# grantjr1842/delayed-streams-modeling

Hardware: AMD Instinct MI355X
Metric: real-time stream throughput, stt-1b-en_fr @ bs=64 per GPU (Mimi encode + LM decode per 80 ms frame) (higher is better)
Workload: dtype bf16 weights + bf16 KV, f32 activations as three exact bf16 pieces, f32 accumulate (v_mfma_f32_16x16x32_bf16); 1 GPU; stt-1b-en_fr batch=64 streaming, ring KV cache full (750 frames), Mimi encode + LM decode HIP path; streams_per_gpu=64, parallelism=replicas x1 (independent stream batches, no per-step collective), streams=encoder stream || 2 LM group stream(s)

## Files before the change

delayed-streams-modeling_amd/csrc/dsm_engine_api.inc:

```

namespace {

template <typename KVT, int HD, int T>
int launch_attn_t(dsm_engine* e, hipStream_t st, float* out, const float* q, const void* k, const void* v,
                  const uint32_t* start_pos, const uint8_t* active, int B, int H, int ctx, int d, const AttnFused& fq) {
  size_t lds = sizeof(float) * ((size_t)T * ctx + 4 * T * HD + 16);
  if ((long)B * H >= 2048 && (size_t)2 * ctx * HD * sizeof(KVT) >= (size_t)256 * 1024) lds += e->attn_lds_pad;
  if (lds > 64 * 1024) {
    static size_t allowed = 0;
    if (lds > allowed) {
      HIPCHK(hipFuncSetAttribute(reinterpret_cast<const void*>(&attn_kernel<KVT, HD, T, 8>), hipFuncAttributeMaxDynamicSharedMemorySize, (int)lds));
      HIPCHK(hipFuncSetAttribute(reinterpret_cast<const void*>(&attn_kernel<KVT, HD, T, 4>), hipFuncAttributeMaxDynamicSharedMemorySize, (int)lds));
      allowed = lds;
    }
  }
  const int tag = e->tag_attn[e->sid(st)];
  if (T == 1 && HD == 64 && ctx <= 32 && e->attn_small) {
    const int ph = e->prof_begin(tag, st);
    hipLaunchKernelGGL((attn_small_kernel<KVT, 64>), dim3((B * H + 3) / 4), dim3(256), 0, st, out, q, reinterpret_cast<const KVT*>(k),
                       reinterpret_cast<const KVT*>(v), start_pos, active, B * H, H, ctx, d, fq);
    e->prof_end(ph, st);
    HIPCHK(hipGetLastError());
    return 0;
  }
  const int ph = e->prof_begin(tag, st);
  const bool unr8 = sizeof(KVT) == 2 && T == 1 && (e->attn_unr == 8 || (e->attn_unr == 0 && HD == 128));
  if (unr8)
    hipLaunchKernelGGL((attn_kernel<KVT, HD, T, 8>), dim3(B * H), dim3(256), lds, st, out, q, reinterpret_cast<const KVT*>(k),
                       reinterpret_cast<const KVT*>(v), start_pos, active, H, ctx, d, e->dev_ts_slot(tag, e->sid(st), 0), fq);
  else
    hipLaunchKernelGGL((attn_kernel<KVT, HD, T, 4>), dim3(B * H), dim3(256), lds, st, out, q, reinterpret_cast<const KVT*>(k),
                       reinterpret_cast<const KVT*>(v), start_pos, active, H, ctx, d, e->dev_ts_slot(tag, e->sid(st), 0), fq);
  e->prof_end(ph, st);
  HIPCHK(hipGetLastError());
  return 0;
}

template <typename KVT>
int launch_attn(dsm_engine* e, hipStream_t st, float* out, const float* q, const void* k, const void* v,
                const uint32_t* start_pos, const uint8_t* active, int B, int H, int hd, int T, int ctx, int d,
                const AttnFused& fq) {
#define DSM_ATTN(HDv, Tv) \
  if (hd == HDv && T == Tv) return launch_attn_t<KVT, HDv, Tv>(e, st, out, q, k, v, start_pos, active, B, H, ctx, d, fq);
  DSM_ATTN(32, 1) DSM_ATTN(64, 1) DSM_ATTN(128, 1) DSM_ATTN(32, 2) DSM_ATTN(64, 2) DSM_ATTN(128, 2)
#undef DSM_ATTN
  e->set_error("unsupported attention shape head_dim=%d T=%d (head_dim must be 32, 64 or 128; T 1 or 2)", hd, T);
  return DSM_ERR_INVALID;
}

int make_stream(dsm_engine* e, hipStream_t* st, int prio, int kind) {
  const int n = e->enc_cus;
  if (n <= 0 || n >= 32 || (kind == 2 && !e->lm_cus_excl)) {
    HIPCHK(hipStreamCreateWithPriority(st, hipStreamNonBlocking, prio));
    return 0;
  }
  uint32_t mask[8];
  for (int w = 0; w < 8; ++w) {
    uint32_t m = 0;
    for (int b = 0; b < 32; ++b) {
      const int cu = (32 * w + b) / 8;
      if ((kind == 1) == (cu < n)) m |= 1u << b;
    }
    mask[w] = m;
  }
  HIPCHK(hipExtStreamCreateWithCUMask(st, 8, mask));
  return 0;
}

int run_norm(dsm_engine* e, hipStream_t st, float* y, const float* x, const float* w, const float* b, int rows, int d,
             int rms) {
  hipLaunchKernelGGL(row_norm_kernel, dim3(rows), dim3(256), 0, st, y, x, w, b, rows, d,
                     rms ? 1e-8f : 1e-5f, rms);
  HIPCHK(hipGetLastError());
  return 0;
}

template <typename WT, typename KVT>
int transformer_forward(dsm_engine* e, hipStream_t st, const TransformerW& w, TransformerState& s, float* x, float* xn,
                        float* q, float* att, float* ff, int B, int T, const uint8_t* d_mask, float* final_out,
                        RowMap final_map, const float* post_norm_w = nullptr, float* post_norm_out = nullptr, int phase = 0,
                        const CaState* ca = nullptr, bool head_done = false) {
  const dsm_transformer_config& c = w.cfg;
  const int d = c.d_model, H = c.num_heads, hd = d / H, M = B * T;
  const float eps = c.norm == 1 ? 1e-8f : 1e-5f;
  if (phase != 2 && !head_done) {
    hipLaunchKernelGGL(kv_builder_kernel, dim3(B), dim3(64), 0, st, s.pos, s.idx, d_mask, s.start_pos, s.widx,
                       c.positional_embedding == 1 ? s.rope_cs : (float*)nullptr, w.inv_freq, B, T, c.context, hd,
                       w.rope_pos_before ? 1 : 0);
    HIPCHK(hipGetLastError());
// ... 1525 lines not shown
```

delayed-streams-modeling_amd/csrc/dsm_kernels.h:

```cpp
#pragma once
#include <hip/hip_runtime.h>
#include <stdint.h>
#include "dsm_numerics.h"
#include "dsm_sampling.h"

typedef float f32x4 __attribute__((ext_vector_type(4)));
typedef short dsm_bf16x8 __attribute__((ext_vector_type(8)));

__device__ __forceinline__ float wave_sum64(float v) {
#pragma unroll
  for (int off = 32; off >= 1; off >>= 1) v = v + __shfl_xor(v, off, 64);
  return v;
}

enum { EPI_STORE = 0, EPI_QKV = 1, EPI_GATE = 2, EPI_RVQ = 3 };

struct RowMap {
  long bstride;
  int rpb;
  int ld;
  int toff;
  __host__ __device__ long off(int m) const { return (long)(m / rpb) * bstride + (long)((m % rpb) + toff) * ld; }
};

struct GemmArgs {
  const float* X;
  RowMap xmap;
  const void* W;
  int Kpad, K, N, M;
  int nt_stride;
  int wpacked;
  int w_ntiles;
  int wg_cols;
  const float* bias;
  const float* scale;
  const float* res;
  RowMap rmap;
  float* Y;
  RowMap ymap;
  float* Y2;
  RowMap y2map;
  int act;
  int vec;
  int d, hd, H, T, ctx;
  void* kcache;
  void* vcache;
  const uint32_t* widx;
  const float* rope_cs;
  const uint8_t* active;
  float* pval;
  uint32_t* pidx;
  float* ws;
  int ws_ntiles;
  int defer_reduce;
  int chunk_loop;
  const float* norm_w;
  const float* norm_b;
  float* norm_out;
  float norm_eps;
  int norm_rms;
  int wk_hint;
  const float* pre_norm_w;
  const float* pre_norm_b;
  float pre_norm_eps;
  int pre_norm_rms;
  unsigned long long* ts;
};

template <typename WT>
__device__ __forceinline__ const WT* dsm_wbase(const GemmArgs& a, const WT* W, int n0, int r, int q) {
  if (sizeof(WT) == 2 && a.wpacked) return W + ((long)(n0 >> 4) * (a.Kpad >> 5)) * 512 + (q * 16 + r) * 8;
  return W + (long)(n0 + r) * a.Kpad + 8 * q;
}
template <typename WT>
__device__ __forceinline__ int dsm_wstep(const GemmArgs& a) { return (sizeof(WT) == 2 && a.wpacked) ? 16 : 1; }

__device__ __forceinline__ void launch_stamp_begin(unsigned long long* ts) {
  if (!ts || threadIdx.x != 0) return;
  const unsigned lin = blockIdx.x + gridDim.x * (blockIdx.y + gridDim.y * blockIdx.z);
  if (lin < 128) atomicMin(&ts[0], wall_clock64());
}
__device__ __forceinline__ void launch_stamp_end(unsigned long long* ts) {
  if (!ts || threadIdx.x != 0) return;
  const unsigned total = gridDim.x * gridDim.y * gridDim.z;
  const unsigned lin = blockIdx.x + gridDim.x * (blockIdx.y + gridDim.y * blockIdx.z);
  if (lin + 512 >= total) atomicMax(&ts[1], wall_clock64());
}

template <typename WT>
__device__ __forceinline__ void load_w8(const WT* p, float (&o)[8]);
template <>
__device__ __forceinline__ void load_w8<uint16_t>(const uint16_t* p, float (&o)[8]) {
  uint4 v = *reinterpret_cast<const uint4*>(p);
  o[0] = __uint_as_float(v.x << 16); o[1] = __uint_as_float(v.x & 0xFFFF0000u);
  o[2] = __uint_as_float(v.y << 16); o[3] = __uint_as_float(v.y & 0xFFFF0000u);
  o[4] = __uint_as_float(v.z << 16); o[5] = __uint_as_float(v.z & 0xFFFF0000u);
  o[6] = __uint_as_float(v.w << 16); o[7] = __uint_as_float(v.w & 0xFFFF0000u);
}
template <>
__device__ __forceinline__ void load_w8<float>(const float* p, float (&o)[8]) {
  float4 a = *reinterpret_cast<const float4*>(p);
  float4 b = *reinterpret_cast<const float4*>(p + 4);
  o[0] = a.x; o[1] = a.y; o[2] = a.z; o[3] = a.w; o[4] = b.x; o[5] = b.y; o[6] = b.z; o[7] = b.w;
}

template <typename KVT>
struct Raw8;
typedef unsigned int dsm_u32x4 __attribute__((ext_vector_type(4)));
typedef float dsm_f32x4v __attribute__((ext_vector_type(4)));
template <>
struct Raw8<uint16_t> {
  uint4 v;
  __device__ __forceinline__ void load(const uint16_t* p) { v = *reinterpret_cast<const uint4*>(p); }
  __device__ __forceinline__ void load_nt(const uint16_t* p) {
    const dsm_u32x4 t = __builtin_nontemporal_load(reinterpret_cast<const dsm_u32x4*>(p));
    v = make_uint4(t[0], t[1], t[2], t[3]);
  }
  __device__ __forceinline__ void unpack(float (&o)[8]) const {
    o[0] = __uint_as_float(v.x << 16); o[1] = __uint_as_float(v.x & 0xFFFF0000u);
    o[2] = __uint_as_float(v.y << 16); o[3] = __uint_as_float(v.y & 0xFFFF0000u);
    o[4] = __uint_as_float(v.z << 16); o[5] = __uint_as_float(v.z & 0xFFFF0000u);
    o[6] = __uint_as_float(v.w << 16); o[7] = __uint_as_float(v.w & 0xFFFF0000u);
  }
};
template <>
struct Raw8<float> {
  float4 a, b;
  __device__ __forceinline__ void load(const float* p) {
    a = *reinterpret_cast<const float4*>(p);
    b = *reinterpret_cast<const float4*>(p + 4);
  }
  __device__ __forceinline__ void load_nt(const float* p) {
    const dsm_f32x4v t0 = __builtin_nontemporal_load(reinterpret_cast<const dsm_f32x4v*>(p));
    const dsm_f32x4v t1 = __builtin_nontemporal_load(reinterpret_cast<const dsm_f32x4v*>(p + 4));
    a = make_float4(t0[0], t0[1], t0[2], t0[3]);
    b = make_float4(t1[0], t1[1], t1[2], t1[3]);
  }
  __device__ __forceinline__ void unpack(float (&o)[8]) const {
    o[0] = a.x; o[1] = a.y; o[2] = a.z; o[3] = a.w; o[4] = b.x; o[5] = b.y; o[6] = b.z; o[7] = b.w;
  }
};

__device__ __forceinline__ void store_kv(uint16_t* p, float v) { *p = dsm_f32_to_bf16(v); }
__device__ __forceinline__ void store_kv(float* p, float v) { *p = v; }

__device__ __forceinline__ void store_kv4(uint16_t* p, const float (&o)[4]) {
  uint2 v;
  v.x = (uint32_t)dsm_f32_to_bf16(o[0]) | ((uint32_t)dsm_f32_to_bf16(o[1]) << 16);
  v.y = (uint32_t)dsm_f32_to_bf16(o[2]) | ((uint32_t)dsm_f32_to_bf16(o[3]) << 16);
  *reinterpret_cast<uint2*>(p) = v;
}
__device__ __forceinline__ void store_kv4(float* p, const float (&o)[4]) {
  *reinterpret_cast<float4*>(p) = make_float4(o[0], o[1], o[2], o[3]);
}

template <typename KVT, int EPI>
__device__ __forceinline__ void epi_store_qkv(const GemmArgs& a, f32x4 v, int m, int n) {
  if (m >= a.M || n >= a.N) return;
  const bool full = a.vec && (n + 3 < a.N);
  if (EPI == EPI_STORE) {
    float o[4];
#pragma unroll
    for (int i = 0; i < 4; ++i) {
      float t = v[i];
      if (n + i < a.N) {
        if (a.bias) t = t + a.bias[n + i];
        if (a.act == 1) t = dsm_gelu_erf(t);
        if (a.scale) t = t * a.scale[n + i];
      }
      o[i] = t;
    }
    if (a.res) {
      const float* rp = a.res + a.rmap.off(m) + n;
      if (full) {
        float4 rv = *reinterpret_cast<const float4*>(rp);
        o[0] = rv.x + o[0]; o[1] = rv.y + o[1]; o[2] = rv.z + o[2]; o[3] = rv.w + o[3];
      } else {
#pragma unroll
        for (int i = 0; i < 4; ++i)
          if (n + i < a.N) o[i] = rp[i] + o[i];
      }
    }
    if (a.Y) {
      float* y = a.Y + a.ymap.off(m) + n;
      if (full) {
        *reinterpret_cast<float4*>(y) = make_float4(o[0], o[1], o[2], o[3]);
      } else {
#pragma unroll
        for (int i = 0; i < 4; ++i)
          if (n + i < a.N) y[i] = o[i];
      }
    }
    if (a.Y2) {
      float* y2 = a.Y2 + a.y2map.off(m) + n;
      if (full) {
        *reinterpret_cast<float4*>(y2) = make_float4(dsm_elu(o[0]), dsm_elu(o[1]), dsm_elu(o[2]), dsm_elu(o[3]));
      } else {
#pragma unroll
        for (int i = 0; i < 4; ++i)
          if (n + i < a.N) y2[i] = dsm_elu(o[i]);
      }
    }
  } else {
    const int part = n / a.d, c = n - part * a.d, h = c / a.hd, i0 = c - h * a.hd;
    const int b = m / a.T;
    float o[4] = {v[0], v[1], v[2], v[3]};
    if (part < 2 && a.rope_cs) {
      const float4 cs = *reinterpret_cast<const float4*>(a.rope_cs + ((long)m * (a.hd / 2) + (i0 >> 1)) * 2);
      const float co[2] = {cs.x, cs.z}, si[2] = {cs.y, cs.w};
#pragma unroll
      for (int p = 0; p < 2; ++p) {
        float x0 = v[2 * p], x1 = v[2 * p + 1];
        float t0 = x0 * co[p], t1 = x1 * si[p], t2 = x0 * si[p], t3 = x1 * co[p];
        o[2 * p] = t0 - t1;
        o[2 * p + 1] = t2 + t3;
      }
    }
    if (part == 0) {
      *reinterpret_cast<float4*>(a.Y + (long)m * a.d + c) = make_float4(o[0], o[1], o[2], o[3]);
    } else if (a.active[b]) {
      KVT* cache = reinterpret_cast<KVT*>(part == 1 ? a.kcache : a.vcache);
      store_kv4(cache + (((long)b * a.H + h) * a.ctx + a.widx[m]) * a.hd + i0, o);
// ... 501 lines not shown
    for (int nt = 0; nt < NT; ++nt) {
      const uint4 w = wv[nt];
      wa[nt][0] = (short)(w.x & 0xFFFF); wa[nt][1] = (short)(w.x >> 16); wa[nt][2] = (short)(w.y & 0xFFFF); wa[nt][3] = (short)(w.y >> 16);
      wa[nt][4] = (short)(w.z & 0xFFFF); wa[nt][5] = (short)(w.z >> 16); wa[nt][6] = (short)(w.w & 0xFFFF); wa[nt][7] = (short)(w.w >> 16);
    }
    {
      const int gn = g + 1 < kb1 ? g + 1 : g;
      xa = *reinterpret_cast<const float4*>(xsrc0 + 32 * gn);
      if (TWO) xb = *reinterpret_cast<const float4*>(xsrc1 + 32 * gn);
#pragma unroll
      for (int nt = 0; nt < NT; ++nt) wv[nt] = *reinterpret_cast<const uint4*>(wrow[nt] + (long)32 * gn * wst);
    }
    __syncthreads();
#pragma unroll
    for (int p = 0; p < 3; ++p)
#pragma unroll
      for (int mt = 0; mt < MT; ++mt) {
        const int row = 16 * mt + r;
        const dsm_bf16x8 xf = *reinterpret_cast<const dsm_bf16x8*>(&Xp[buf][p][0][0] + row * 32 + ((q ^ ((row >> 1) & 3)) * 8));
#pragma unroll
        for (int nt = 0; nt < NT; ++nt) acc[nt][mt] = __builtin_amdgcn_mfma_f32_16x16x32_bf16(wa[nt], xf, acc[nt][mt], 0, 0, 0);
      }
    if (LOOP && ((g & 7) == 7 || g == kb1 - 1)) {
#pragma unroll
      for (int nt = 0; nt < NT; ++nt)
#pragma unroll
        for (int mt = 0; mt < MT; ++mt) {
          tot[nt][mt] = tot[nt][mt] + acc[nt][mt];
          acc[nt][mt] = (f32x4){0.f, 0.f, 0.f, 0.f};
        }
    }
  }
  if (!LOOP) {
#pragma unroll
    for (int nt = 0; nt < NT; ++nt)
#pragma unroll
      for (int mt = 0; mt < MT; ++mt) tot[nt][mt] = (f32x4){0.f, 0.f, 0.f, 0.f} + acc[nt][mt];
  }
  if (chunks > 1) {
    const long ld = (long)a.ws_ntiles * 16;
    const long mpad = (long)((a.M + 15) >> 4) * 16;
#pragma unroll
    for (int mt = 0; mt < MT; ++mt) {
      const int m = m_base + 16 * mt + r;
      if (m >= mpad) continue;
#pragma unroll
      for (int nt = 0; nt < NT; ++nt) {
        const int n = n_base + nt * a.nt_stride + 4 * q;
        *reinterpret_cast<f32x4*>(a.ws + ((long)blockIdx.y * mpad + m) * ld + n) = tot[nt][mt];
      }
    }
    launch_stamp_end(a.ts);
    return;
  }
#pragma unroll
  for (int mt = 0; mt < MT; ++mt) {
    const int m = m_base + 16 * mt + r;
    if (EPI == EPI_GATE) {
      epi_gate(a, tot[0][mt], tot[NT - 1][mt], m, n_base + 4 * q);
    } else {
#pragma unroll
      for (int nt = 0; nt < NT; ++nt) epi_store_qkv<KVT, EPI>(a, tot[nt][mt], m, n_base + nt * a.nt_stride + 4 * q);
    }
  }
  launch_stamp_end(a.ts);
}

__device__ __forceinline__ f32x4 slab_sum(const float* p, long cstride, int chunks) {
  f32x4 t = *reinterpret_cast<const f32x4*>(p);
  for (int c0 = 1; c0 < chunks; c0 += 8) {
    f32x4 v[8];
#pragma unroll
    for (int u = 0; u < 8; ++u) {
      const int c = c0 + u < chunks ? c0 + u : chunks - 1;
      v[u] = *reinterpret_cast<const f32x4*>(p + c * cstride);
    }
#pragma unroll
    for (int u = 0; u < 8; ++u)
      if (c0 + u < chunks) t = t + v[u];
  }
  return t;
}

template <typename KVT, int EPI>
__global__ __launch_bounds__(256) void gemm_reduce_kernel(GemmArgs a, int chunks) {
  launch_stamp_begin(a.ts ? a.ts + 2 : nullptr);
  const int lane = threadIdx.x & 63, wave = threadIdx.x >> 6;
  const int r = lane & 15, q = lane >> 4;
  const int mtiles = (a.M + 15) >> 4;
  const int out_ntiles = (a.N + 15) >> 4;
  const int t = blockIdx.x * 4 + wave;
  if (t >= mtiles * out_ntiles) return;
  const int mtile = t / out_ntiles, ntile = t % out_ntiles;
  constexpr int NT = (EPI == EPI_GATE) ? 2 : 1;
  const long ld = (long)a.ws_ntiles * 16, cstride = (long)mtiles * 16 * ld;
  const int m = mtile * 16 + r, n = ntile * 16 + 4 * q;
  f32x4 tot[NT];
#pragma unroll
  for (int nt = 0; nt < NT; ++nt) {
    tot[nt] = slab_sum(a.ws + (long)m * ld + n + nt * a.nt_stride, cstride, chunks);
  }
  if (EPI == EPI_GATE)
    epi_gate(a, tot[0], tot[NT - 1], m, n);
  else if (EPI == EPI_RVQ)
    epi_rvq(a, tot[0], m, n, ntile, q);
  else
    epi_store_qkv<KVT, EPI>(a, tot[0], m, n);
  launch_stamp_end(a.ts ? a.ts + 2 : nullptr);
}

#include "dsm_gemm_wk.h"

__device__ __forceinline__ void block_row_sums(float& s, float& s2, float* red) {
  const int lane = threadIdx.x & 63, wave = threadIdx.x >> 6;
  s = wave_sum64(s);
  s2 = wave_sum64(s2);
  if (lane == 0) { red[wave] = s; red[4 + wave] = s2; }
  __syncthreads();
  s = ((red[0] + red[1]) + red[2]) + red[3];
  s2 = ((red[4] + red[5]) + red[6]) + red[7];
}

#define DSM_ROW_ITS 4

__device__ __forceinline__ void row_norm_apply(const float4 (&v)[DSM_ROW_ITS], float s, float s2, int d, float eps, int rms,
                                               const float* __restrict__ w, const float* __restrict__ b,
                                               float* __restrict__ out) {
  float mm = 1.f, mean = 0.f, inv = 0.f;
  if (rms) {
    mm = sqrtf(s2 / (float)d + eps);
  } else {
    mean = s / (float)d;
    float var = s2 / (float)d - mean * mean;
    inv = 1.0f / sqrtf(var + eps);
  }
#pragma unroll
  for (int it = 0; it < DSM_ROW_ITS; ++it) {
    const int i = it * 1024 + 4 * (int)threadIdx.x;
    if (i < d) {
      const float4 wv = *reinterpret_cast<const float4*>(w + i);
      float4 o;
      if (rms) {
        o.x = (v[it].x / mm) * wv.x; o.y = (v[it].y / mm) * wv.y; o.z = (v[it].z / mm) * wv.z; o.w = (v[it].w / mm) * wv.w;
      } else {
        const float4 bv = *reinterpret_cast<const float4*>(b + i);
        o.x = ((v[it].x - mean) * inv) * wv.x + bv.x; o.y = ((v[it].y - mean) * inv) * wv.y + bv.y;
        o.z = ((v[it].z - mean) * inv) * wv.z + bv.z; o.w = ((v[it].w - mean) * inv) * wv.w + bv.w;
      }
      *reinterpret_cast<float4*>(out + i) = o;
    }
  }
}

template <int ITS>
__global__ __launch_bounds__(256 * ITS) void gemm_reduce_rows_kernel(GemmArgs a, int chunks) {
  constexpr int RS = ITS == 4 ? 16 : 24;
  __shared__ float red[8];
  __shared__ float carry[2][256];
  launch_stamp_begin(a.ts ? a.ts + 2 : nullptr);
  const int m = blockIdx.x;
  const int d = a.N;
  const int it = threadIdx.x >> 8, t = threadIdx.x & 255;
  const long ld = (long)a.ws_ntiles * 16, cstride = (long)((a.M + 15) >> 4) * 16 * ld;
  const int i = it * 1024 + 4 * t;
  const bool live = i < d;
  const float* p = a.ws + (long)m * ld + (live ? i : 4 * t);
// ... 35 lines not shown
    if (it == k) {
      if (k > 0) { s = carry[0][t]; s2 = carry[1][t]; }
      if (live) {
        s = s + o[0]; s2 = DSM_FMAF(o[0], o[0], s2);
        s = s + o[1]; s2 = DSM_FMAF(o[1], o[1], s2);
        s = s + o[2]; s2 = DSM_FMAF(o[2], o[2], s2);
        s = s + o[3]; s2 = DSM_FMAF(o[3], o[3], s2);
      }
      if (k + 1 < ITS) { carry[0][t] = s; carry[1][t] = s2; }
    }
    if (k + 1 < ITS) __syncthreads();
  }
  if (it == ITS - 1) {
    const int lane = t & 63, wave = t >> 6;
    s = wave_sum64(s);
    s2 = wave_sum64(s2);
    if (lane == 0) { red[wave] = s; red[4 + wave] = s2; }
  }
  __syncthreads();
  s = ((red[0] + red[1]) + red[2]) + red[3];
  s2 = ((red[4] + red[5]) + red[6]) + red[7];
  if (live) {
    float mm = 1.f, mean = 0.f, inv = 0.f;
    if (a.norm_rms) {
      mm = sqrtf(s2 / (float)d + a.norm_eps);
    } else {
      mean = s / (float)d;
      float var = s2 / (float)d - mean * mean;
      inv = 1.0f / sqrtf(var + a.norm_eps);
    }
    float4 r;
    if (a.norm_rms) {
      r.x = (o[0] / mm) * nw4[0]; r.y = (o[1] / mm) * nw4[1]; r.z = (o[2] / mm) * nw4[2]; r.w = (o[3] / mm) * nw4[3];
    } else {
      r.x = ((o[0] - mean) * inv) * nw4[0] + nb4[0]; r.y = ((o[1] - mean) * inv) * nw4[1] + nb4[1];
      r.z = ((o[2] - mean) * inv) * nw4[2] + nb4[2]; r.w = ((o[3] - mean) * inv) * nw4[3] + nb4[3];
    }
    *reinterpret_cast<float4*>(a.norm_out + (long)m * d + i) = r;
  }
  launch_stamp_end(a.ts ? a.ts + 2 : nullptr);
}

__global__ __launch_bounds__(256) void row_norm_kernel(float* __restrict__ y, const float* __restrict__ x,
                                                       const float* __restrict__ w, const float* __restrict__ b, int rows,
                                                       int d, float eps, int rms) {
  __shared__ float red[8];
  const int row = blockIdx.x;
  const float* xr = x + (long)row * d;
  float4 v[DSM_ROW_ITS];
  float s = 0.0f, s2 = 0.0f;
#pragma unroll
  for (int it = 0; it < DSM_ROW_ITS; ++it) {
    const int i = it * 1024 + 4 * (int)threadIdx.x;
    v[it] = make_float4(0.f, 0.f, 0.f, 0.f);
    if (i < d) {
      v[it] = *reinterpret_cast<const float4*>(xr + i);
      s = s + v[it].x; s2 = DSM_FMAF(v[it].x, v[it].x, s2);
      s = s + v[it].y; s2 = DSM_FMAF(v[it].y, v[it].y, s2);
      s = s + v[it].z; s2 = DSM_FMAF(v[it].z, v[it].z, s2);
      s = s + v[it].w; s2 = DSM_FMAF(v[it].w, v[it].w, s2);
    }
  }
  block_row_sums(s, s2, red);
  row_norm_apply(v, s, s2, d, eps, rms, w, b, y + (long)row * d);
}

struct AttnFused {
  const float* ws;
  long ld, cstride;
  int chunks;
  const float* rope_cs;
  const uint32_t* widx;
  int nt;
  int q_only;
};

template <typename KVT, int HD, int T, int UNRB = 8>
__global__ __launch_bounds__(256, 4) void attn_kernel(float* __restrict__ out, const float* __restrict__ qbuf,
                                                   const KVT* __restrict__ kcache, const KVT* __restrict__ vcache,
                                                   const uint32_t* __restrict__ start_pos,
                                                   const uint8_t* __restrict__ active, int H, int ctx, int d,
                                                   unsigned long long* __restrict__ ts, AttnFused fq) {
  constexpr int NW = 4, LPK = HD / 8, G = 64 / LPK;
  extern __shared__ __attribute__((aligned(16))) float lds[];
  const int b = blockIdx.x / H, h = blockIdx.x % H;
  const bool ts_first = ts && threadIdx.x == 0 && blockIdx.x < 256;
  const bool ts_last = ts && threadIdx.x == 0 && blockIdx.x + 1024 >= gridDim.x;
  if (ts_first) atomicMin(&ts[0], wall_clock64());
  if (!active[b]) {
    if (ts_last) atomicMax(&ts[1], wall_clock64());
    return;
  }
  const int tid = threadIdx.x, lane = tid & 63, wave = tid >> 6;
  const int g = lane / LPK, li = lane % LPK;
  float* sc = lds;
  float* red = lds + T * ctx;
  float* scratch = red + NW * T * HD;

  const uint32_t sp = start_pos[b];
  const long e1 = (long)sp + T - 1;
  const int nvalid = (int)((e1 + 1 < (long)ctx) ? e1 + 1 : ctx);
  const float scale = (float)(1.0 / sqrt((double)HD));

  const KVT* Kb = kcache + ((long)b * H + h) * ctx * HD;
  const KVT* Vb = vcache + ((long)b * H + h) * ctx * HD;
  if (T == 1 && fq.ws) {
    if (tid < (fq.q_only ? HD / 4 : 3 * HD / 4)) {
      const int part = tid / (HD / 4), i0 = 4 * (tid % (HD / 4));
      const f32x4 v = slab_sum(fq.ws + (long)b * fq.ld + part * d + h * HD + i0, fq.cstride, fq.chunks);
      float o[4] = {v[0], v[1], v[2], v[3]};
      if (part < 2 && fq.rope_cs) {
        const float4 cs = *reinterpret_cast<const float4*>(fq.rope_cs + ((long)b * (HD / 2) + (i0 >> 1)) * 2);
        const float co[2] = {cs.x, cs.z}, si[2] = {cs.y, cs.w};
#pragma unroll
        for (int p = 0; p < 2; ++p) {
          float x0 = v[2 * p], x1 = v[2 * p + 1];
          float t0 = x0 * co[p], t1 = x1 * si[p], t2 = x0 * si[p], t3 = x1 * co[p];
          o[2 * p] = t0 - t1;
          o[2 * p + 1] = t2 + t3;
        }
      }
      if (part == 0) {
        red[i0] = o[0]; red[i0 + 1] = o[1]; red[i0 + 2] = o[2]; red[i0 + 3] = o[3];
      } else {
        KVT* row = const_cast<KVT*>(part == 1 ? Kb : Vb) + (long)fq.widx[b] * HD + i0;
        store_kv4(row, o);
      }
    }
    __syncthreads();
  }
  float qv[T][8];
#pragma unroll
  for (int t = 0; t < T; ++t) {
    if (T == 1 && fq.ws) {
#pragma unroll
      for (int dd = 0; dd < 8; ++dd) qv[t][dd] = red[8 * li + dd];
    } else {
      const float* qp = qbuf + ((long)(b * T + t)) * d + h * HD + 8 * li;
      float4 q0 = *reinterpret_cast<const float4*>(qp), q1 = *reinterpret_cast<const float4*>(qp + 4);
      qv[t][0] = q0.x; qv[t][1] = q0.y; qv[t][2] = q0.z; qv[t][3] = q0.w;
      qv[t][4] = q1.x; qv[t][5] = q1.y; qv[t][6] = q1.z; qv[t][7] = q1.w;
    }
  }
  if (T == 1 && fq.ws) __syncthreads();

  constexpr int UNR = sizeof(KVT) == 2 ? UNRB : 4;
  constexpr int STEP = UNR * NW * G;
  const int jlast = nvalid - 1;
  const int last_slot = (int)(e1 % ctx);
  Raw8<KVT> ra[UNR], rb[UNR];
#define DSM_ISSUE(R, BASE, J0)                                                        \
  _Pragma("unroll") for (int u = 0; u < UNR; ++u) {                                    \
    const int jj = min((J0) + u * NW * G + g, jlast);                                  \
    if (fq.nt) R[u].load_nt(BASE + (long)jj * HD + 8 * li);                            \
    else R[u].load(BASE + (long)jj * HD + 8 * li);                                     \
  }
#define DSM_SCORES(R, J0)                                                              \
  _Pragma("unroll") for (int u = 0; u < UNR; ++u) {                                    \
    const int j = (J0) + u * NW * G + g;                                               \
    int delta = last_slot - min(j, jlast);  \
    delta += (delta < 0) ? ctx : 0;                                                    \
    float kv[8];                                                                       \
    R[u].unpack(kv);                                                                   \
    _Pragma("unroll") for (int t = 0; t < T; ++t) {                                    \
      float p = 0.0f;                                                                  \
      _Pragma("unroll") for (int dd = 0; dd < 8; ++dd) p = DSM_FMAF(qv[t][dd], kv[dd], p); \
      _Pragma("unroll") for (int off = LPK / 2; off >= 1; off >>= 1) p = p + __shfl_xor(p, off, 64); \
      if (li == 0 && j < nvalid) sc[t * ctx + j] = (delta >= T - 1 - t) ? p * scale : -DSM_INF_F; \
    }                                                                                  \
  }
  {
    int j0 = wave * G;
    DSM_ISSUE(ra, Kb, j0)
    while (j0 < nvalid) {
      DSM_ISSUE(rb, Kb, j0 + STEP)
      DSM_SCORES(ra, j0)
      j0 += STEP;
      if (j0 >= nvalid) break;
      DSM_ISSUE(ra, Kb, j0 + STEP)
      DSM_SCORES(rb, j0)
      j0 += STEP;
    }
  }
  DSM_ISSUE(ra, Vb, wave * G)
  __syncthreads();

  float lsum[T];
#pragma unroll
  for (int t = 0; t < T; ++t) {
    float m = -DSM_INF_F;
    for (int j = tid; j < nvalid; j += 256) m = fmaxf(m, sc[t * ctx + j]);
#pragma unroll
    for (int off = 32; off >= 1; off >>= 1) m = fmaxf(m, __shfl_xor(m, off, 64));
    if (lane == 0) scratch[wave] = m;
    __syncthreads();
    m = fmaxf(fmaxf(scratch[0], scratch[1]), fmaxf(scratch[2], scratch[3]));
    __syncthreads();
    float tp = 0.0f;
    for (int j = tid; j < nvalid; j += 256) {
      float p = dsm_expf(sc[t * ctx + j] - m);
      sc[t * ctx + j] = p;
      tp = tp + p;
    }
    tp = wave_sum64(tp);
    if (lane == 0) scratch[4 + wave] = tp;
    __syncthreads();
    lsum[t] = ((scratch[4] + scratch[5]) + scratch[6]) + scratch[7];
    __syncthreads();
  }

  float acc[T][8];
#pragma unroll
  for (int t = 0; t < T; ++t)
#pragma unroll
    for (int dd = 0; dd < 8; ++dd) acc[t][dd] = 0.0f;
#define DSM_PV(R, J0)                                                                  \
  _Pragma("unroll") for (int u = 0; u < UNR; ++u) {  \
    const int j = (J0) + u * NW * G + g;                                               \
    float vv[8];                                                                       \
    R[u].unpack(vv);                                                                   \
    _Pragma("unroll") for (int t = 0; t < T; ++t) {                                    \
       \
      const float wgt = (j < nvalid) ? sc[t * ctx + j] / lsum[t] : 0.0f;               \
      _Pragma("unroll") for (int dd = 0; dd < 8; ++dd) acc[t][dd] = DSM_FMAF(wgt, vv[dd], acc[t][dd]); \
    }                                                                                  \
  }
  {
    int j0 = wave * G;
    while (j0 < nvalid) {
      DSM_ISSUE(rb, Vb, j0 + STEP)
      DSM_PV(ra, j0)
      j0 += STEP;
      if (j0 >= nvalid) break;
      DSM_ISSUE(ra, Vb, j0 + STEP)
      DSM_PV(rb, j0)
      j0 += STEP;
    }
  }
#undef DSM_ISSUE
#undef DSM_SCORES
#undef DSM_PV
#pragma unroll
  for (int t = 0; t < T; ++t)
#pragma unroll
    for (int dd = 0; dd < 8; ++dd) {
      float v = acc[t][dd];
#pragma unroll
      for (int off = 32; off >= LPK; off >>= 1) v = v + __shfl_xor(v, off, 64);
      acc[t][dd] = v;
    }
  if (g == 0) {
#pragma unroll
    for (int t = 0; t < T; ++t)
#pragma unroll
      for (int dd = 0; dd < 8; ++dd) red[(wave * T + t) * HD + 8 * li + dd] = acc[t][dd];
  }
  __syncthreads();
  for (int i = tid; i < T * HD; i += 256) {
    int t = i / HD, dd = i % HD;
    float tot = ((red[(0 * T + t) * HD + dd] + red[(1 * T + t) * HD + dd]) + red[(2 * T + t) * HD + dd]) +
                red[(3 * T + t) * HD + dd];
    out[((long)(b * T + t)) * d + h * HD + dd] = tot;
  }
  if (ts_last) atomicMax(&ts[1], wall_clock64());
}

template <typename KVT, int HD>
__global__ __launch_bounds__(256) void attn_small_kernel(float* __restrict__ out, const float* __restrict__ qbuf,
                                                         const KVT* __restrict__ kcache, const KVT* __restrict__ vcache,
                                                         const uint32_t* __restrict__ start_pos, const uint8_t* __restrict__ active,
                                                         int BH, int H, int ctx, int d, AttnFused fq) {
  static_assert(HD == 64, "one lane group of 8 lanes per key");
  constexpr int LPK = HD / 8;
  __shared__ __attribute__((aligned(16))) float lds_all[4][32 + HD];
  const int tid = threadIdx.x, lane = tid & 63, wave = tid >> 6;
  const int unit = blockIdx.x * 4 + wave;
  const int uc = unit < BH ? unit : BH - 1;
  const int b = uc / H, h = uc % H;
  const bool on = unit < BH && active[b];
  float* sc = lds_all[wave];
  float* qs = sc + 32;
  const int g = lane / LPK, li = lane % LPK;
  const uint32_t sp = start_pos[b];
  const long e1 = (long)sp;
  const int nvalid = (int)((e1 + 1 < (long)ctx) ? e1 + 1 : ctx);
  const float scale = (float)(1.0 / sqrt((double)HD));
  const KVT* Kb = kcache + ((long)b * H + h) * ctx * HD;
  const KVT* Vb = vcache + ((long)b * H + h) * ctx * HD;
  if (fq.ws) {
    if (on && lane < (fq.q_only ? HD / 4 : 3 * HD / 4)) {
      const int part = lane / (HD / 4), i0 = 4 * (lane % (HD / 4));
      const f32x4 v = slab_sum(fq.ws + (long)b * fq.ld + part * d + h * HD + i0, fq.cstride, fq.chunks);
      float o[4] = {v[0], v[1], v[2], v[3]};
      if (part < 2 && fq.rope_cs) {
        const float4 cs = *reinterpret_cast<const float4*>(fq.rope_cs + ((long)b * (HD / 2) + (i0 >> 1)) * 2);
        const float co[2] = {cs.x, cs.z}, si[2] = {cs.y, cs.w};
#pragma unroll
        for (int p = 0; p < 2; ++p) {
          float x0 = v[2 * p], x1 = v[2 * p + 1];
          float t0 = x0 * co[p], t1 = x1 * si[p], t2 = x0 * si[p], t3 = x1 * co[p];
          o[2 * p] = t0 - t1;
          o[2 * p + 1] = t2 + t3;
        }
      }
      if (part == 0) {
        qs[i0] = o[0]; qs[i0 + 1] = o[1]; qs[i0 + 2] = o[2]; qs[i0 + 3] = o[3];
      } else {
        KVT* row = const_cast<KVT*>(part == 1 ? Kb : Vb) + (long)fq.widx[b] * HD + i0;
        store_kv4(row, o);
      }
    }
    __syncthreads();
  }
  if (!on) return;
  float qv[8];
  if (fq.ws) {
#pragma unroll
    for (int dd = 0; dd < 8; ++dd) qv[dd] = qs[8 * li + dd];
  } else {
// ... 793 lines not shown
```

Before: 1824 x realtime (stream-seconds of audio per wall second).

## Prefetch K before QKV fusion, DPP row sums, batched score stores, prenormalized softmax

The attention decode kernel now issues the first K-cache loads before the fused QKV/RoPE prologue. It stages the freshly written K row in LDS so the in-flight load of that slot can be patched instead of racing the global write. Shuffle-based group reductions become DPP row reductions, and score stores are coalesced so one lane per unroll writes. Softmax weights are divided by the sum once in LDS rather than per PV FMA, and two V batches are prefetched before the barrier. This hides global latency and trims ALU/shuffle work, at the cost of extra LDS, more registers and more complex correctness conditions around the ring slot.

```diff
diff --git a/delayed-streams-modeling_amd/csrc/dsm_engine_api.inc b/delayed-streams-modeling_amd/csrc/dsm_engine_api.inc
--- a/delayed-streams-modeling_amd/csrc/dsm_engine_api.inc
+++ b/delayed-streams-modeling_amd/csrc/dsm_engine_api.inc
@@ -4,7 +4,7 @@
 template <typename KVT, int HD, int T>
 int launch_attn_t(dsm_engine* e, hipStream_t st, float* out, const float* q, const void* k, const void* v,
                   const uint32_t* start_pos, const uint8_t* active, int B, int H, int ctx, int d, const AttnFused& fq) {
-  size_t lds = sizeof(float) * ((size_t)T * ctx + 4 * T * HD + 16);
+  size_t lds = HD * sizeof(KVT) + sizeof(float) * ((size_t)T * ctx + 4 * T * HD + 16);
   if ((long)B * H >= 2048 && (size_t)2 * ctx * HD * sizeof(KVT) >= (size_t)256 * 1024) lds += e->attn_lds_pad;
   if (lds > 64 * 1024) {
     static size_t allowed = 0;
diff --git a/delayed-streams-modeling_amd/csrc/dsm_kernels.h b/delayed-streams-modeling_amd/csrc/dsm_kernels.h
--- a/delayed-streams-modeling_amd/csrc/dsm_kernels.h
+++ b/delayed-streams-modeling_amd/csrc/dsm_kernels.h
@@ -11,6 +11,25 @@
 #pragma unroll
   for (int off = 32; off >= 1; off >>= 1) v = v + __shfl_xor(v, off, 64);
   return v;
+}
+
+template <int CTRL, int BANKS = 0xf>
+__device__ __forceinline__ float dpp_lane(float p) {
+  return __int_as_float(__builtin_amdgcn_update_dpp(0, __float_as_int(p), CTRL, 0xf, BANKS, false));
+}
+template <int LPK>
+__device__ __forceinline__ float row_sum(float p) {
+  static_assert(LPK == 4 || LPK == 8 || LPK == 16, "row_sum: 4, 8 or 16 lanes per group");
+  if (LPK == 16) {
+    p = p + dpp_lane<0x128>(p);
+    p = p + dpp_lane<0x124>(p);
+  } else if (LPK == 8) {
+    const float lo = p + dpp_lane<0x104, 0x5>(p);
+    p = lo + dpp_lane<0x114, 0xa>(p);
+  }
+  p = p + dpp_lane<0x4e>(p);
+  p = p + dpp_lane<0xb1>(p);
+  return p;
 }
 
 enum { EPI_STORE = 0, EPI_QKV = 1, EPI_GATE = 2, EPI_RVQ = 3 };
@@ -1017,8 +1036,9 @@
   }
   const int tid = threadIdx.x, lane = tid & 63, wave = tid >> 6;
   const int g = lane / LPK, li = lane % LPK;
-  float* sc = lds;
-  float* red = lds + T * ctx;
+  KVT* krow = reinterpret_cast<KVT*>(lds);
+  float* sc = lds + HD * (int)sizeof(KVT) / 4;
+  float* red = sc + T * ctx;
   float* scratch = red + NW * T * HD;
 
   const uint32_t sp = start_pos[b];
@@ -1028,6 +1048,23 @@
 
   const KVT* Kb = kcache + ((long)b * H + h) * ctx * HD;
   const KVT* Vb = vcache + ((long)b * H + h) * ctx * HD;
+  constexpr int UNR = sizeof(KVT) == 2 ? UNRB : 4;
+  constexpr int STEP = UNR * NW * G;
+  const int jlast = nvalid - 1;
+  const int last_slot = (int)(e1 % ctx);
+  Raw8<KVT> ra[UNR], rb[UNR];
+#define DSM_ISSUE(R, BASE, J0)                                                        \
+  if (fq.nt) {                                                                         \
+    _Pragma("unroll") for (int u = 0; u < UNR; ++u)                                    \
+      R[u].load_nt(BASE + (long)min((J0) + u * NW * G + g, jlast) * HD + 8 * li);      \
+  } else {                                                                             \
+    _Pragma("unroll") for (int u = 0; u < UNR; ++u)                                    \
+      R[u].load(BASE + (long)min((J0) + u * NW * G + g, jlast) * HD + 8 * li);         \
+  }
+  const bool early_k = T == 1 && UNR == 8 && fq.ws && !fq.q_only;
+  if (early_k) {
+    DSM_ISSUE(ra, Kb, wave * G)
+  }
   if (T == 1 && fq.ws) {
     if (tid < (fq.q_only ? HD / 4 : 3 * HD / 4)) {
       const int part = tid / (HD / 4), i0 = 4 * (tid % (HD / 4));
@@ -1049,6 +1086,7 @@
       } else {
         KVT* row = const_cast<KVT*>(part == 1 ? Kb : Vb) + (long)fq.widx[b] * HD + i0;
         store_kv4(row, o);
+        if (part == 1) store_kv4(krow + i0, o);
       }
     }
     __syncthreads();
@@ -1068,34 +1106,41 @@
   }
   if (T == 1 && fq.ws) __syncthreads();
 
-  constexpr int UNR = sizeof(KVT) == 2 ? UNRB : 4;
-  constexpr int STEP = UNR * NW * G;
-  const int jlast = nvalid - 1;
-  const int last_slot = (int)(e1 % ctx);
-  Raw8<KVT> ra[UNR], rb[UNR];
-#define DSM_ISSUE(R, BASE, J0)                                                        \
-  _Pragma("unroll") for (int u = 0; u < UNR; ++u) {                                    \
-    const int jj = min((J0) + u * NW * G + g, jlast);                                  \
-    if (fq.nt) R[u].load_nt(BASE + (long)jj * HD + 8 * li);                            \
-    else R[u].load(BASE + (long)jj * HD + 8 * li);                                     \
-  }
+  constexpr bool ONE_STORE = UNR <= LPK;
 #define DSM_SCORES(R, J0)                                                              \
-  _Pragma("unroll") for (int u = 0; u < UNR; ++u) {                                    \
-    const int j = (J0) + u * NW * G + g;                                               \
-    int delta = last_slot - min(j, jlast);  \
-    delta += (delta < 0) ? ctx : 0;                                                    \
-    float kv[8];                                                                       \
-    R[u].unpack(kv);                                                                   \
-    _Pragma("unroll") for (int t = 0; t < T; ++t) {                                    \
-      float p = 0.0f;                                                                  \
-      _Pragma("unroll") for (int dd = 0; dd < 8; ++dd) p = DSM_FMAF(qv[t][dd], kv[dd], p); \
-      _Pragma("unroll") for (int off = LPK / 2; off >= 1; off >>= 1) p = p + __shfl_xor(p, off, 64); \
-      if (li == 0 && j < nvalid) sc[t * ctx + j] = (delta >= T - 1 - t) ? p * scale : -DSM_INF_F; \
+  {                                                                                    \
+    float mine[T];                                                                     \
+    _Pragma("unroll") for (int u = 0; u < UNR; ++u) {                                  \
+      float kv[8];                                                                     \
+      R[u].unpack(kv);                                                                 \
+      _Pragma("unroll") for (int t = 0; t < T; ++t) {                                  \
+        float p = 0.0f;                                                                \
+        _Pragma("unroll") for (int dd = 0; dd < 8; ++dd) p = DSM_FMAF(qv[t][dd], kv[dd], p); \
+        p = row_sum<LPK>(p);                                                           \
+        if (ONE_STORE) mine[t] = (u == 0 || li == u) ? p : mine[t];                    \
+        else mine[t] = p;                                                              \
+      }                                                                                \
+      if (!ONE_STORE || u == UNR - 1) {                                                \
+        const int j = (J0) + (ONE_STORE ? li : u) * NW * G + g;                        \
+        int delta = last_slot - min(j, jlast);  \
+        delta += (delta < 0) ? ctx : 0;                                                \
+        if ((ONE_STORE ? li < UNR : li == 0) && j < nvalid) {                          \
+          _Pragma("unroll") for (int t = 0; t < T; ++t)                                \
+            sc[t * ctx + j] = (delta >= T - 1 - t) ? mine[t] * scale : -DSM_INF_F;     \
+        }                                                                              \
+      }                                                                                \
     }                                                                                  \
   }
   {
     int j0 = wave * G;
-    DSM_ISSUE(ra, Kb, j0)
+    if (early_k) {
+      const int kslot = (int)fq.widx[b];
+#pragma unroll
+      for (int u = 0; u < UNR; ++u)
+        if (min(j0 + u * NW * G + g, jlast) == kslot) ra[u].load(krow + 8 * li);
+    } else {
+      DSM_ISSUE(ra, Kb, j0)
+    }
     while (j0 < nvalid) {
       DSM_ISSUE(rb, Kb, j0 + STEP)
       DSM_SCORES(ra, j0)
@@ -1107,9 +1152,9 @@
     }
   }
   DSM_ISSUE(ra, Vb, wave * G)
-  __syncthreads();
-
-  float lsum[T];
+  DSM_ISSUE(rb, Vb, wave * G + STEP)
+  __syncthreads();
+
 #pragma unroll
   for (int t = 0; t < T; ++t) {
     float m = -DSM_INF_F;
@@ -1129,7 +1174,8 @@
     tp = wave_sum64(tp);
     if (lane == 0) scratch[4 + wave] = tp;
     __syncthreads();
-    lsum[t] = ((scratch[4] + scratch[5]) + scratch[6]) + scratch[7];
+    const float lsum = ((scratch[4] + scratch[5]) + scratch[6]) + scratch[7];
+    for (int j = tid; j < nvalid; j += 256) sc[t * ctx + j] = sc[t * ctx + j] / lsum;
     __syncthreads();
   }
 
@@ -1145,20 +1191,21 @@
     R[u].unpack(vv);                                                                   \
     _Pragma("unroll") for (int t = 0; t < T; ++t) {                                    \
        \
-      const float wgt = (j < nvalid) ? sc[t * ctx + j] / lsum[t] : 0.0f;               \
+      const float wgt = (j < nvalid) ? sc[t * ctx + j] : 0.0f;                         \
       _Pragma("unroll") for (int dd = 0; dd < 8; ++dd) acc[t][dd] = DSM_FMAF(wgt, vv[dd], acc[t][dd]); \
     }                                                                                  \
   }
   {
     int j0 = wave * G;
     while (j0 < nvalid) {
-      DSM_ISSUE(rb, Vb, j0 + STEP)
       DSM_PV(ra, j0)
       j0 += STEP;
       if (j0 >= nvalid) break;
       DSM_ISSUE(ra, Vb, j0 + STEP)
       DSM_PV(rb, j0)
       j0 += STEP;
+      if (j0 >= nvalid) break;
+      DSM_ISSUE(rb, Vb, j0 + STEP)
     }
   }
 #undef DSM_ISSUE
```

Measured after the change: 1780 x realtime (stream-seconds of audio per wall second). 2.4% lower.

## Prefetch K cache and QKV slab before active check in attention kernel

Applied to the files above, without the earlier changes.

The first K-cache tile and the first split-K QKV slab chunks are now loaded at kernel entry, before the active check and the fused QKV reduction. A new K row that lands in the first tile is patched in from an LDS staging copy, so the early load cannot see a stale value. The softmax now normalises the scores in LDS once, removing the per-element division in the PV loop, and drops two block barriers per row by giving each row its own scratch slots. The aim is to hide the global-load latency behind the slab reduction. In exchange the kernel uses more registers and issues loads for inactive batches, and the staged-row patching is subtle.

```diff
diff --git a/delayed-streams-modeling_amd/csrc/dsm_kernels.h b/delayed-streams-modeling_amd/csrc/dsm_kernels.h
--- a/delayed-streams-modeling_amd/csrc/dsm_kernels.h
+++ b/delayed-streams-modeling_amd/csrc/dsm_kernels.h
@@ -122,6 +122,11 @@
     o[4] = __uint_as_float(v.z << 16); o[5] = __uint_as_float(v.z & 0xFFFF0000u);
     o[6] = __uint_as_float(v.w << 16); o[7] = __uint_as_float(v.w & 0xFFFF0000u);
   }
+  __device__ static __forceinline__ void stage4(uint32_t* s, int i0, const float (&o)[4]) {
+    s[i0 / 2] = (uint32_t)dsm_f32_to_bf16(o[0]) | ((uint32_t)dsm_f32_to_bf16(o[1]) << 16);
+    s[i0 / 2 + 1] = (uint32_t)dsm_f32_to_bf16(o[2]) | ((uint32_t)dsm_f32_to_bf16(o[3]) << 16);
+  }
+  __device__ __forceinline__ void load_staged(const uint32_t* s, int li) { v = make_uint4(s[4 * li], s[4 * li + 1], s[4 * li + 2], s[4 * li + 3]); }
 };
 template <>
 struct Raw8<float> {
@@ -138,6 +143,15 @@
   }
   __device__ __forceinline__ void unpack(float (&o)[8]) const {
     o[0] = a.x; o[1] = a.y; o[2] = a.z; o[3] = a.w; o[4] = b.x; o[5] = b.y; o[6] = b.z; o[7] = b.w;
+  }
+  __device__ static __forceinline__ void stage4(uint32_t* s, int i0, const float (&o)[4]) {
+#pragma unroll
+    for (int k = 0; k < 4; ++k) s[i0 + k] = __float_as_uint(o[k]);
+  }
+  __device__ __forceinline__ void load_staged(const uint32_t* s, int li) {
+    const uint32_t* q = s + 8 * li;
+    a = make_float4(__uint_as_float(q[0]), __uint_as_float(q[1]), __uint_as_float(q[2]), __uint_as_float(q[3]));
+    b = make_float4(__uint_as_float(q[4]), __uint_as_float(q[5]), __uint_as_float(q[6]), __uint_as_float(q[7]));
   }
 };
 
@@ -805,6 +819,36 @@
   return t;
 }
 
+struct SlabHead {
+  f32x4 t, v[8];
+};
+__device__ __forceinline__ void slab_issue(SlabHead& s, const float* p, long cstride, int chunks) {
+  s.t = *reinterpret_cast<const f32x4*>(p);
+#pragma unroll
+  for (int u = 0; u < 8; ++u) {
+    const int c = 1 + u < chunks ? 1 + u : chunks - 1;
+    s.v[u] = *reinterpret_cast<const f32x4*>(p + c * cstride);
+  }
+}
+__device__ __forceinline__ f32x4 slab_finish(const SlabHead& s, const float* p, long cstride, int chunks) {
+  f32x4 t = s.t;
+#pragma unroll
+  for (int u = 0; u < 8; ++u)
+    if (1 + u < chunks) t = t + s.v[u];
+  for (int c0 = 9; c0 < chunks; c0 += 8) {
+    f32x4 v[8];
+#pragma unroll
+    for (int u = 0; u < 8; ++u) {
+      const int c = c0 + u < chunks ? c0 + u : chunks - 1;
+      v[u] = *reinterpret_cast<const f32x4*>(p + c * cstride);
+    }
+#pragma unroll
+    for (int u = 0; u < 8; ++u)
+      if (c0 + u < chunks) t = t + v[u];
+  }
+  return t;
+}
+
 template <typename KVT, int EPI>
 __global__ __launch_bounds__(256) void gemm_reduce_kernel(GemmArgs a, int chunks) {
   launch_stamp_begin(a.ts ? a.ts + 2 : nullptr);
@@ -1006,35 +1050,60 @@
                                                    const uint8_t* __restrict__ active, int H, int ctx, int d,
                                                    unsigned long long* __restrict__ ts, AttnFused fq) {
   constexpr int NW = 4, LPK = HD / 8, G = 64 / LPK;
+  constexpr int UNR = sizeof(KVT) == 2 ? UNRB : 4;
+  constexpr int STEP = UNR * NW * G;
   extern __shared__ __attribute__((aligned(16))) float lds[];
   const int b = blockIdx.x / H, h = blockIdx.x % H;
   const bool ts_first = ts && threadIdx.x == 0 && blockIdx.x < 256;
   const bool ts_last = ts && threadIdx.x == 0 && blockIdx.x + 1024 >= gridDim.x;
   if (ts_first) atomicMin(&ts[0], wall_clock64());
-  if (!active[b]) {
-    if (ts_last) atomicMax(&ts[1], wall_clock64());
-    return;
-  }
   const int tid = threadIdx.x, lane = tid & 63, wave = tid >> 6;
   const int g = lane / LPK, li = lane % LPK;
   float* sc = lds;
   float* red = lds + T * ctx;
   float* scratch = red + NW * T * HD;
-
+  uint32_t* kstage = reinterpret_cast<uint32_t*>(red + HD);
+
+  const KVT* Kb = kcache + ((long)b * H + h) * ctx * HD;
+  const KVT* Vb = vcache + ((long)b * H + h) * ctx * HD;
+  const bool fused = T == 1 && fq.ws != nullptr, fused_kv = fused && !fq.q_only;
+
+  const uint8_t act = active[b];
   const uint32_t sp = start_pos[b];
+  const uint32_t wrow = fused_kv ? fq.widx[b] : 0u;
+  const bool slab_thr = fused && tid < (fq.q_only ? HD / 4 : 3 * HD / 4);
+  const int part = tid / (HD / 4), i0 = 4 * (tid % (HD / 4));
+  const float* slab = fused ? fq.ws + (long)b * fq.ld + part * d + h * HD + i0 : nullptr;
+  SlabHead sh;
+  float4 cs = make_float4(0.f, 0.f, 0.f, 0.f);
+  if (slab_thr) {
+    slab_issue(sh, slab, fq.cstride, fq.chunks);
+    if (part < 2 && fq.rope_cs) cs = *reinterpret_cast<const float4*>(fq.rope_cs + ((long)b * (HD / 2) + (i0 >> 1)) * 2);
+  }
+  Raw8<KVT> ra[UNR], rb[UNR];
+#define DSM_ISSUE(R, BASE, J0, JMAX)    \
+  if (fq.nt) {                                                                         \
+    _Pragma("unroll") for (int u = 0; u < UNR; ++u)                                    \
+      R[u].load_nt(BASE + (long)min((J0) + u * NW * G + g, (JMAX)) * HD + 8 * li);     \
+  } else {                                                                             \
+    _Pragma("unroll") for (int u = 0; u < UNR; ++u)                                    \
+      R[u].load(BASE + (long)min((J0) + u * NW * G + g, (JMAX)) * HD + 8 * li);        \
+  }
+  DSM_ISSUE(ra, Kb, wave * G, ctx - 1)
+  __builtin_amdgcn_sched_barrier(0);
+  if (!act) {
+    if (ts_last) atomicMax(&ts[1], wall_clock64());
+    return;
+  }
+
   const long e1 = (long)sp + T - 1;
   const int nvalid = (int)((e1 + 1 < (long)ctx) ? e1 + 1 : ctx);
   const float scale = (float)(1.0 / sqrt((double)HD));
-
-  const KVT* Kb = kcache + ((long)b * H + h) * ctx * HD;
-  const KVT* Vb = vcache + ((long)b * H + h) * ctx * HD;
-  if (T == 1 && fq.ws) {
-    if (tid < (fq.q_only ? HD / 4 : 3 * HD / 4)) {
-      const int part = tid / (HD / 4), i0 = 4 * (tid % (HD / 4));
-      const f32x4 v = slab_sum(fq.ws + (long)b * fq.ld + part * d + h * HD + i0, fq.cstride, fq.chunks);
+  if (fused) {
+    if (slab_thr) {
+      const f32x4 v = slab_finish(sh, slab, fq.cstride, fq.chunks);
       float o[4] = {v[0], v[1], v[2], v[3]};
       if (part < 2 && fq.rope_cs) {
-        const float4 cs = *reinterpret_cast<const float4*>(fq.rope_cs + ((long)b * (HD / 2) + (i0 >> 1)) * 2);
         const float co[2] = {cs.x, cs.z}, si[2] = {cs.y, cs.w};
 #pragma unroll
         for (int p = 0; p < 2; ++p) {
@@ -1047,8 +1116,9 @@
       if (part == 0) {
         red[i0] = o[0]; red[i0 + 1] = o[1]; red[i0 + 2] = o[2]; red[i0 + 3] = o[3];
       } else {
-        KVT* row = const_cast<KVT*>(part == 1 ? Kb : Vb) + (long)fq.widx[b] * HD + i0;
+        KVT* row = const_cast<KVT*>(part == 1 ? Kb : Vb) + (long)wrow * HD + i0;
         store_kv4(row, o);
+        if (part == 1) Raw8<KVT>::stage4(kstage, i0, o);
       }
     }
     __syncthreads();
@@ -1056,7 +1126,7 @@
   float qv[T][8];
 #pragma unroll
   for (int t = 0; t < T; ++t) {
-    if (T == 1 && fq.ws) {
+    if (fused) {
 #pragma unroll
       for (int dd = 0; dd < 8; ++dd) qv[t][dd] = red[8 * li + dd];
     } else {
@@ -1066,19 +1136,9 @@
       qv[t][4] = q1.x; qv[t][5] = q1.y; qv[t][6] = q1.z; qv[t][7] = q1.w;
     }
   }
-  if (T == 1 && fq.ws) __syncthreads();
-
-  constexpr int UNR = sizeof(KVT) == 2 ? UNRB : 4;
-  constexpr int STEP = UNR * NW * G;
+
   const int jlast = nvalid - 1;
   const int last_slot = (int)(e1 % ctx);
-  Raw8<KVT> ra[UNR], rb[UNR];
-#define DSM_ISSUE(R, BASE, J0)                                                        \
-  _Pragma("unroll") for (int u = 0; u < UNR; ++u) {                                    \
-    const int jj = min((J0) + u * NW * G + g, jlast);                                  \
-    if (fq.nt) R[u].load_nt(BASE + (long)jj * HD + 8 * li);                            \
-    else R[u].load(BASE + (long)jj * HD + 8 * li);                                     \
-  }
 #define DSM_SCORES(R, J0)                                                              \
   _Pragma("unroll") for (int u = 0; u < UNR; ++u) {                                    \
     const int j = (J0) + u * NW * G + g;                                               \
@@ -1095,31 +1155,37 @@
   }
   {
     int j0 = wave * G;
-    DSM_ISSUE(ra, Kb, j0)
+    DSM_ISSUE(rb, Kb, j0 + STEP, jlast)
+    if (fused_kv && wrow < (uint32_t)STEP) {
+      Raw8<KVT> knew;
+      knew.load_staged(kstage, li);
+#pragma unroll
+      for (int u = 0; u < UNR; ++u)
+        if (min(j0 + u * NW * G + g, ctx - 1) == (int)wrow) ra[u] = knew;
+    }
     while (j0 < nvalid) {
-      DSM_ISSUE(rb, Kb, j0 + STEP)
       DSM_SCORES(ra, j0)
       j0 += STEP;
       if (j0 >= nvalid) break;
-      DSM_ISSUE(ra, Kb, j0 + STEP)
+      DSM_ISSUE(ra, Kb, j0 + STEP, jlast)
       DSM_SCORES(rb, j0)
       j0 += STEP;
-    }
-  }
-  DSM_ISSUE(ra, Vb, wave * G)
-  __syncthreads();
-
-  float lsum[T];
+      if (j0 >= nvalid) break;
+      DSM_ISSUE(rb, Kb, j0 + STEP, jlast)
+    }
+  }
+  DSM_ISSUE(ra, Vb, wave * G, jlast)
+  __syncthreads();
+
 #pragma unroll
   for (int t = 0; t < T; ++t) {
     float m = -DSM_INF_F;
     for (int j = tid; j < nvalid; j += 256) m = fmaxf(m, sc[t * ctx + j]);
 #pragma unroll
     for (int off = 32; off >= 1; off >>= 1) m = fmaxf(m, __shfl_xor(m, off, 64));
-    if (lane == 0) scratch[wave] = m;
+    if (lane == 0) scratch[8 * t + wave] = m;
     __syncthreads();
-    m = fmaxf(fmaxf(scratch[0], scratch[1]), fmaxf(scratch[2], scratch[3]));
-    __syncthreads();
+    m = fmaxf(fmaxf(scratch[8 * t], scratch[8 * t + 1]), fmaxf(scratch[8 * t + 2], scratch[8 * t + 3]));
     float tp = 0.0f;
     for (int j = tid; j < nvalid; j += 256) {
       float p = dsm_expf(sc[t * ctx + j] - m);
@@ -1127,11 +1193,12 @@
       tp = tp + p;
     }
     tp = wave_sum64(tp);
-    if (lane == 0) scratch[4 + wave] = tp;
+    if (lane == 0) scratch[8 * t + 4 + wave] = tp;
     __syncthreads();
-    lsum[t] = ((scratch[4] + scratch[5]) + scratch[6]) + scratch[7];
-    __syncthreads();
-  }
+    const float lsum = ((scratch[8 * t + 4] + scratch[8 * t + 5]) + scratch[8 * t + 6]) + scratch[8 * t + 7];
+    for (int j = tid; j < nvalid; j += 256) sc[t * ctx + j] = sc[t * ctx + j] / lsum;
+  }
+  __syncthreads();
 
   float acc[T][8];
 #pragma unroll
@@ -1145,18 +1212,18 @@
     R[u].unpack(vv);                                                                   \
     _Pragma("unroll") for (int t = 0; t < T; ++t) {                                    \
        \
-      const float wgt = (j < nvalid) ? sc[t * ctx + j] / lsum[t] : 0.0f;               \
+      const float wgt = (j < nvalid) ? sc[t * ctx + j] : 0.0f;                         \
       _Pragma("unroll") for (int dd = 0; dd < 8; ++dd) acc[t][dd] = DSM_FMAF(wgt, vv[dd], acc[t][dd]); \
     }                                                                                  \
   }
   {
     int j0 = wave * G;
     while (j0 < nvalid) {
-      DSM_ISSUE(rb, Vb, j0 + STEP)
+      DSM_ISSUE(rb, Vb, j0 + STEP, jlast)
       DSM_PV(ra, j0)
       j0 += STEP;
       if (j0 >= nvalid) break;
-      DSM_ISSUE(ra, Vb, j0 + STEP)
+      DSM_ISSUE(ra, Vb, j0 + STEP, jlast)
       DSM_PV(rb, j0)
       j0 += STEP;
     }
```

Measured after the change: 1797 x realtime (stream-seconds of audio per wall second) before, 1783 x realtime (stream-seconds of audio per wall second) after. Within noise of the previous version (-0.8%).
